# hrpan/tetris_mcts

Hardware: NVIDIA H100
Metric: mcts_sims_per_sec (higher is better)
Workload: dtype f32

## Files before the change

### tetris_mcts_b200/csrc/valuenet_tc.cuh

```cuda
#pragma once
#include <cuda_fp16.h>
#include "gmma.cuh"
#include "search_dev.cuh"
#include "valuenet_simt.cuh"

namespace b200 {

constexpr float TC_SCALE_A = 16.f, TC_SCALE_W = 64.f, TC_UNSCALE = 1.f / 1024.f;

__device__ __forceinline__ void wgmma_n64(float (&d)[32], uint64_t adesc, uint64_t bdesc, uint32_t accumulate) {
    asm volatile(
        "{\n.reg .pred p;\nsetp.ne.b32 p, %34, 0;\n"
        "wgmma.mma_async.sync.aligned.m64n64k16.f32.f16.f16 {"
        "%0,%1,%2,%3,%4,%5,%6,%7,%8,%9,%10,%11,%12,%13,%14,%15,"
        "%16,%17,%18,%19,%20,%21,%22,%23,%24,%25,%26,%27,%28,%29,%30,%31"
        "}, %32, %33, p, 1, 1, 0, 0;\n}"
        : "+f"(d[0]), "+f"(d[1]), "+f"(d[2]), "+f"(d[3]), "+f"(d[4]), "+f"(d[5]), "+f"(d[6]), "+f"(d[7]),
          "+f"(d[8]), "+f"(d[9]), "+f"(d[10]), "+f"(d[11]), "+f"(d[12]), "+f"(d[13]), "+f"(d[14]), "+f"(d[15]),
          "+f"(d[16]), "+f"(d[17]), "+f"(d[18]), "+f"(d[19]), "+f"(d[20]), "+f"(d[21]), "+f"(d[22]), "+f"(d[23]),
          "+f"(d[24]), "+f"(d[25]), "+f"(d[26]), "+f"(d[27]), "+f"(d[28]), "+f"(d[29]), "+f"(d[30]), "+f"(d[31])
        : "l"(adesc), "l"(bdesc), "r"(accumulate));
}
__device__ __forceinline__ void wgmma_n96(float (&d)[48], uint64_t adesc, uint64_t bdesc, uint32_t accumulate) {
    asm volatile(
        "{\n.reg .pred p;\nsetp.ne.b32 p, %50, 0;\n"
        "wgmma.mma_async.sync.aligned.m64n96k16.f32.f16.f16 {"
        "%0,%1,%2,%3,%4,%5,%6,%7,%8,%9,%10,%11,%12,%13,%14,%15,"
        "%16,%17,%18,%19,%20,%21,%22,%23,%24,%25,%26,%27,%28,%29,%30,%31,"
        "%32,%33,%34,%35,%36,%37,%38,%39,%40,%41,%42,%43,%44,%45,%46,%47"
        "}, %48, %49, p, 1, 1, 0, 0;\n}"
        : "+f"(d[0]), "+f"(d[1]), "+f"(d[2]), "+f"(d[3]), "+f"(d[4]), "+f"(d[5]), "+f"(d[6]), "+f"(d[7]),
          "+f"(d[8]), "+f"(d[9]), "+f"(d[10]), "+f"(d[11]), "+f"(d[12]), "+f"(d[13]), "+f"(d[14]), "+f"(d[15]),
          "+f"(d[16]), "+f"(d[17]), "+f"(d[18]), "+f"(d[19]), "+f"(d[20]), "+f"(d[21]), "+f"(d[22]), "+f"(d[23]),
          "+f"(d[24]), "+f"(d[25]), "+f"(d[26]), "+f"(d[27]), "+f"(d[28]), "+f"(d[29]), "+f"(d[30]), "+f"(d[31]),
          "+f"(d[32]), "+f"(d[33]), "+f"(d[34]), "+f"(d[35]), "+f"(d[36]), "+f"(d[37]), "+f"(d[38]), "+f"(d[39]),
          "+f"(d[40]), "+f"(d[41]), "+f"(d[42]), "+f"(d[43]), "+f"(d[44]), "+f"(d[45]), "+f"(d[46]), "+f"(d[47])
        : "l"(adesc), "l"(bdesc), "r"(accumulate));
}
__device__ __forceinline__ void wgmma_n128(float (&d)[64], uint64_t adesc, uint64_t bdesc, uint32_t accumulate) {
    asm volatile(
        "{\n.reg .pred p;\nsetp.ne.b32 p, %66, 0;\n"
        "wgmma.mma_async.sync.aligned.m64n128k16.f32.f16.f16 {"
        "%0,%1,%2,%3,%4,%5,%6,%7,%8,%9,%10,%11,%12,%13,%14,%15,"
        "%16,%17,%18,%19,%20,%21,%22,%23,%24,%25,%26,%27,%28,%29,%30,%31,"
        "%32,%33,%34,%35,%36,%37,%38,%39,%40,%41,%42,%43,%44,%45,%46,%47,"
        "%48,%49,%50,%51,%52,%53,%54,%55,%56,%57,%58,%59,%60,%61,%62,%63"
        "}, %64, %65, p, 1, 1, 0, 0;\n}"
        : "+f"(d[0]), "+f"(d[1]), "+f"(d[2]), "+f"(d[3]), "+f"(d[4]), "+f"(d[5]), "+f"(d[6]), "+f"(d[7]),
          "+f"(d[8]), "+f"(d[9]), "+f"(d[10]), "+f"(d[11]), "+f"(d[12]), "+f"(d[13]), "+f"(d[14]), "+f"(d[15]),
          "+f"(d[16]), "+f"(d[17]), "+f"(d[18]), "+f"(d[19]), "+f"(d[20]), "+f"(d[21]), "+f"(d[22]), "+f"(d[23]),
          "+f"(d[24]), "+f"(d[25]), "+f"(d[26]), "+f"(d[27]), "+f"(d[28]), "+f"(d[29]), "+f"(d[30]), "+f"(d[31]),
          "+f"(d[32]), "+f"(d[33]), "+f"(d[34]), "+f"(d[35]), "+f"(d[36]), "+f"(d[37]), "+f"(d[38]), "+f"(d[39]),
          "+f"(d[40]), "+f"(d[41]), "+f"(d[42]), "+f"(d[43]), "+f"(d[44]), "+f"(d[45]), "+f"(d[46]), "+f"(d[47]),
          "+f"(d[48]), "+f"(d[49]), "+f"(d[50]), "+f"(d[51]), "+f"(d[52]), "+f"(d[53]), "+f"(d[54]), "+f"(d[55]),
          "+f"(d[56]), "+f"(d[57]), "+f"(d[58]), "+f"(d[59]), "+f"(d[60]), "+f"(d[61]), "+f"(d[62]), "+f"(d[63])
        : "l"(adesc), "l"(bdesc), "r"(accumulate));
}
__device__ __forceinline__ void wgmma_n256(float (&d)[128], uint64_t adesc, uint64_t bdesc, uint32_t accumulate) {
    asm volatile(
        "{\n.reg .pred p;\nsetp.ne.b32 p, %130, 0;\n"
        "wgmma.mma_async.sync.aligned.m64n256k16.f32.f16.f16 {"
        "%0,%1,%2,%3,%4,%5,%6,%7,%8,%9,%10,%11,%12,%13,%14,%15,"
        "%16,%17,%18,%19,%20,%21,%22,%23,%24,%25,%26,%27,%28,%29,%30,%31,"
        "%32,%33,%34,%35,%36,%37,%38,%39,%40,%41,%42,%43,%44,%45,%46,%47,"
        "%48,%49,%50,%51,%52,%53,%54,%55,%56,%57,%58,%59,%60,%61,%62,%63,"
        "%64,%65,%66,%67,%68,%69,%70,%71,%72,%73,%74,%75,%76,%77,%78,%79,"
        "%80,%81,%82,%83,%84,%85,%86,%87,%88,%89,%90,%91,%92,%93,%94,%95,"
        "%96,%97,%98,%99,%100,%101,%102,%103,%104,%105,%106,%107,%108,%109,%110,%111,"
        "%112,%113,%114,%115,%116,%117,%118,%119,%120,%121,%122,%123,%124,%125,%126,%127"
        "}, %128, %129, p, 1, 1, 0, 0;\n}"
        : "+f"(d[0]), "+f"(d[1]), "+f"(d[2]), "+f"(d[3]), "+f"(d[4]), "+f"(d[5]), "+f"(d[6]), "+f"(d[7]),
          "+f"(d[8]), "+f"(d[9]), "+f"(d[10]), "+f"(d[11]), "+f"(d[12]), "+f"(d[13]), "+f"(d[14]), "+f"(d[15]),
          "+f"(d[16]), "+f"(d[17]), "+f"(d[18]), "+f"(d[19]), "+f"(d[20]), "+f"(d[21]), "+f"(d[22]), "+f"(d[23]),
          "+f"(d[24]), "+f"(d[25]), "+f"(d[26]), "+f"(d[27]), "+f"(d[28]), "+f"(d[29]), "+f"(d[30]), "+f"(d[31]),
          "+f"(d[32]), "+f"(d[33]), "+f"(d[34]), "+f"(d[35]), "+f"(d[36]), "+f"(d[37]), "+f"(d[38]), "+f"(d[39]),
          "+f"(d[40]), "+f"(d[41]), "+f"(d[42]), "+f"(d[43]), "+f"(d[44]), "+f"(d[45]), "+f"(d[46]), "+f"(d[47]),
          "+f"(d[48]), "+f"(d[49]), "+f"(d[50]), "+f"(d[51]), "+f"(d[52]), "+f"(d[53]), "+f"(d[54]), "+f"(d[55]),
          "+f"(d[56]), "+f"(d[57]), "+f"(d[58]), "+f"(d[59]), "+f"(d[60]), "+f"(d[61]), "+f"(d[62]), "+f"(d[63]),
          "+f"(d[64]), "+f"(d[65]), "+f"(d[66]), "+f"(d[67]), "+f"(d[68]), "+f"(d[69]), "+f"(d[70]), "+f"(d[71]),
          "+f"(d[72]), "+f"(d[73]), "+f"(d[74]), "+f"(d[75]), "+f"(d[76]), "+f"(d[77]), "+f"(d[78]), "+f"(d[79]),
          "+f"(d[80]), "+f"(d[81]), "+f"(d[82]), "+f"(d[83]), "+f"(d[84]), "+f"(d[85]), "+f"(d[86]), "+f"(d[87]),
          "+f"(d[88]), "+f"(d[89]), "+f"(d[90]), "+f"(d[91]), "+f"(d[92]), "+f"(d[93]), "+f"(d[94]), "+f"(d[95]),
          "+f"(d[96]), "+f"(d[97]), "+f"(d[98]), "+f"(d[99]), "+f"(d[100]), "+f"(d[101]), "+f"(d[102]), "+f"(d[103]),
          "+f"(d[104]), "+f"(d[105]), "+f"(d[106]), "+f"(d[107]), "+f"(d[108]), "+f"(d[109]), "+f"(d[110]), "+f"(d[111]),
          "+f"(d[112]), "+f"(d[113]), "+f"(d[114]), "+f"(d[115]), "+f"(d[116]), "+f"(d[117]), "+f"(d[118]), "+f"(d[119]),
          "+f"(d[120]), "+f"(d[121]), "+f"(d[122]), "+f"(d[123]), "+f"(d[124]), "+f"(d[125]), "+f"(d[126]), "+f"(d[127])
        : "l"(adesc), "l"(bdesc), "r"(accumulate));
}
__device__ __forceinline__ void split2(float x0, float x1, uint32_t &hi, uint32_t &lo) {
    const __half2 h = __floats2half2_rn(x0, x1);
    const float2 f = __half22float2(h);
    const __half2 l = __floats2half2_rn(x0 - f.x, x1 - f.y);
    hi = *reinterpret_cast<const uint32_t *>(&h); lo = *reinterpret_cast<const uint32_t *>(&l);
}

constexpr int TCC_WGS = 4;
constexpr int TCC_THREADS = TCC_WGS * 128;
constexpr int TCC_R = 144;
constexpr int TCC_WBLOCK = 2 * 2 * 96 * 16;
constexpr int TCC_WBYTES = 6 * TCC_WBLOCK;
constexpr int TCC_W1BYTES = 2 * 64 * 16;
constexpr int TCC_RUN = 4;
constexpr int TCC_ASLOT = 2 * 4 * TCC_R * 16;
constexpr int TCC_IMROWS = 192;
constexpr int TCC_IMSLOT = 2 * TCC_IMROWS * 16;
constexpr int TCC_OFF_W2 = 0;
constexpr int TCC_OFF_W3 = TCC_OFF_W2 + TCC_WBYTES;
constexpr int TCC_OFF_W1 = TCC_OFF_W3 + TCC_WBYTES;
constexpr int TCC_OFF_A1 = TCC_OFF_W1 + TCC_W1BYTES;
constexpr int TCC_OFF_IM = TCC_OFF_A1 + TCC_WGS * TCC_ASLOT;
constexpr int TCC_OFF_BIAS = TCC_OFF_IM + TCC_WGS * TCC_IMSLOT;
constexpr int TCC_OFF_KEY = TCC_OFF_BIAS + 96 * 4;
constexpr int TCC_SMEM = TCC_OFF_KEY + TCC_WGS * 32 * 4;
constexpr int ACT3_KCHUNKS = 224;
static_assert(TCC_SMEM <= 227 * 1024, "k_tc_conv shared memory");

struct TcWeights {
    const uint8_t *wc1;
    const uint8_t *wc2, *wc3;
    const uint8_t *wfc;
};

__device__ __forceinline__ size_t act3_off(int split, int n_tiles, int ridx, int kchunk) {
    return ((((size_t)split * n_tiles + (ridx >> 7)) * ACT3_KCHUNKS + kchunk) * 128 + (ridx & 127)) * 16;
}

__device__ __forceinline__ void issue_conv_layer(float (&d)[48], uint32_t a_addr, uint32_t w_addr) {
    const uint64_t a0 = gmma_desc(a_addr, TCC_R * 16, 128), b0 = gmma_desc(w_addr, 96 * 16, 128);
#pragma unroll
    for (int dy = 0; dy < 3; ++dy) {
#pragma unroll
        for (int h = 0; h < 2; ++h) {
            const uint32_t a_hi = 2 * h * TCC_R + dy * 8, a_lo = a_hi + 4 * TCC_R;
            const uint32_t b_hi = (dy * 2 + h) * (TCC_WBLOCK / 16), b_lo = b_hi + 2 * 96;
            wgmma_n96(d, a0 + a_hi, b0 + b_hi, (dy | h) ? 1u : 0u);
            wgmma_n96(d, a0 + a_hi, b0 + b_lo, 1u);
            wgmma_n96(d, a0 + a_lo, b0 + b_hi, 1u);
        }
    }
}

__device__ __forceinline__ void build_im2col3(uint8_t *im, const uint32_t *tab, int wt) {
    for (int p = wt; p < TCC_R; p += 128) {
        const int y = p >> 3, x = p & 7;
        uint32_t hv[9];
#pragma unroll
        for (int dy = 0; dy < 3; ++dy) {
            const uint32_t rw = tab[y + dy] >> x;
#pragma unroll
            for (int dx = 0; dx < 3; ++dx)
                hv[dy * 3 + dx] = ((rw >> dx) & 1u) * 0x3C00u | ((rw >> (16 + dx)) & 1u) * 0xBC00u;
        }
        *reinterpret_cast<uint4 *>(im + p * 16) =
            make_uint4(hv[0] | (hv[1] << 16), hv[2] | (hv[3] << 16), hv[4] | (hv[5] << 16), hv[6] | (hv[7] << 16));
        *reinterpret_cast<uint32_t *>(im + TCC_IMROWS * 16 + p * 16) = hv[8];
    }
}

__global__ void __launch_bounds__(TCC_THREADS, 1)
k_tc_conv(NetWeights W, TcWeights TW, const uint2 *req, const int32_t *n_req_ptr, const int32_t *first_ptr, const uint32_t *keys, int M, uint8_t *act3,
          int n_tiles, unsigned long long *prof) {
    extern __shared__ __align__(128) uint8_t smem[];
    float *sB = reinterpret_cast<float *>(smem + TCC_OFF_BIAS);
    const int t = threadIdx.x, wg = t >> 7, wt = t & 127, w = wt >> 5, lane = t & 31;
    for (int i = t; i < TCC_WBYTES / 16; i += TCC_THREADS) {
        reinterpret_cast<uint4 *>(smem + TCC_OFF_W2)[i] = reinterpret_cast<const uint4 *>(TW.wc2)[i];
        reinterpret_cast<uint4 *>(smem + TCC_OFF_W3)[i] = reinterpret_cast<const uint4 *>(TW.wc3)[i];
    }
    for (int i = t; i < TCC_W1BYTES / 16; i += TCC_THREADS) reinterpret_cast<uint4 *>(smem + TCC_OFF_W1)[i] = reinterpret_cast<const uint4 *>(TW.wc1)[i];
    for (int i = t; i < (TCC_OFF_BIAS - TCC_OFF_A1) / 16; i += TCC_THREADS) reinterpret_cast<uint4 *>(smem + TCC_OFF_A1)[i] = make_uint4(0, 0, 0, 0);
    if (t < 32) { sB[t] = W.b1[t] * TC_SCALE_A; sB[32 + t] = W.b2[t] * TC_SCALE_A; sB[64 + t] = W.b3[t] * TC_SCALE_A; }
    fence_async_smem();
    __syncthreads();
    const int first = first_ptr ? *first_ptr : 0;
    const int n_req = *n_req_ptr - first;
    const int n_workers = (int)gridDim.x * TCC_WGS, wid = (int)blockIdx.x * TCC_WGS + wg;
    const int n_runs = (n_req + TCC_RUN - 1) / TCC_RUN;
    int n_local = 0;
    for (int run = wid; run < n_runs; run += n_workers) n_local += min(TCC_RUN, n_req - run * TCC_RUN);
    auto board_of = [&](int i) -> int { return first + ((i / TCC_RUN) * n_workers + wid) * TCC_RUN + (i % TCC_RUN); };
    uint8_t *act = smem + TCC_OFF_A1 + wg * TCC_ASLOT, *im = smem + TCC_OFF_IM + wg * TCC_IMSLOT;
    uint32_t *sKey = reinterpret_cast<uint32_t *>(smem + TCC_OFF_KEY) + wg * 32;
    const uint32_t s_act = smem_u32(act), s_im = smem_u32(im);
    const uint32_t s_w1 = smem_u32(smem + TCC_OFF_W1), s_w2 = smem_u32(smem + TCC_OFF_W2), s_w3 = smem_u32(smem + TCC_OFF_W3);
    const int qd = lane & 3, rl = lane >> 2;
    constexpr float K23 = TC_UNSCALE * TC_SCALE_A, K1 = TC_SCALE_A / TC_SCALE_W;
    constexpr int SPLIT = 4 * TCC_R * 16;
    const bool do_prof = prof && blockIdx.x == 0 && t == 0;
    long long pacc[4] = {0, 0, 0, 0}, ptick = clock64();
    auto prof_t = [&](int k) { if (do_prof) { const long long n = clock64(); pacc[k] += n - ptick; ptick = n; } };
    auto fetch = [&](int i) -> uint32_t {
        if (i >= n_local || lane >= 12) return 0u;
        const uint2 rq = req[board_of(i)];
        return keys[((size_t)rq.x * M + (rq.y & 0x0fffffffu)) * KEY_WORDS + lane];
    };
    uint32_t kw = w == 0 ? fetch(0) : 0u;
    for (int i = 0; i < n_local; ++i) {
        const int ridx = board_of(i);
        if (w == 0) {
            const uint32_t rowpair = __shfl_sync(0xffffffffu, kw, (lane >> 1) & 15), pcs = __shfl_sync(0xffffffffu, kw, 10);
            uint32_t tab = (rowpair >> ((lane & 1) * 16)) & 0x3ffu;
#pragma unroll
            for (int k = 0; k < 4; ++k) {
                const uint32_t cell = (pcs >> (8 * k)) & 0xffu, pr = (cell * 205u) >> 11, pcol = cell - pr * 10u;
                tab |= (pr == (uint32_t)lane ? 1u : 0u) << (16 + pcol);
            }
            kw = fetch(i + 1);
            if (lane < 20) sKey[lane] = tab;
        }
        wg_sync(wg);
        build_im2col3(im, sKey, wt);
        fence_async_smem();
        wg_sync(wg);
        prof_t(0);
#pragma unroll 1
        for (int mt = 0; mt < 3; ++mt) {
            float d[32];
#pragma unroll
            for (int k = 0; k < 32; ++k) d[k] = 0.f;
            wgmma_fence();
            wgmma_n64(d, gmma_desc(s_im + mt * 1024, TCC_IMROWS * 16, 128), gmma_desc(s_w1, 64 * 16, 128), 0u);
            wgmma_commit();
            wgmma_wait<0>();
            fence_regs(d);
#pragma unroll
            for (int h = 0; h < 2; ++h) {
                const int r = mt * 64 + 16 * w + 8 * h + rl;
                if (r < TCC_R) {
#pragma unroll
                    for (int j = 0; j < 4; ++j) {
                        const int c = 8 * j + 2 * qd;
                        const float o0 = fmaxf(fmaf(d[4 * (j + 4) + 2 * h] + d[4 * j + 2 * h], K1, sB[c]), 0.f);
                        const float o1 = fmaxf(fmaf(d[4 * (j + 4) + 2 * h + 1] + d[4 * j + 2 * h + 1], K1, sB[c + 1]), 0.f);
                        uint32_t hi, lo;
                        split2(o0, o1, hi, lo);
                        uint8_t *dst = act + (j * TCC_R + r) * 16 + qd * 4;
                        *reinterpret_cast<uint32_t *>(dst) = hi;
                        *reinterpret_cast<uint32_t *>(dst + SPLIT) = lo;
                    }
                }
            }
        }
        fence_async_smem();
        wg_sync(wg);
        prof_t(1);
#pragma unroll 1
        for (int layer = 0; layer < 2; ++layer) {
            const float *bias = sB + 32 * (layer + 1);
#pragma unroll 1
            for (int mt = 0; mt < 2; ++mt) {
                float d[48];
#pragma unroll
                for (int k = 0; k < 48; ++k) d[k] = 0.f;
                wgmma_fence();
                issue_conv_layer(d, s_act + mt * 1024, layer ? s_w3 : s_w2);
                wgmma_commit();
                wgmma_wait<0>();
                fence_regs(d);
#pragma unroll
                for (int h = 0; h < 2; ++h) {
                    const int y = mt * 8 + 2 * w + h, x = rl;
#pragma unroll
                    for (int j = 0; j < 4; ++j) {
                        float o[2];
#pragma unroll
                        for (int e = 0; e < 2; ++e) {
                            const int k = 4 * j + 2 * h + e;
                            const float s1 = __shfl_down_sync(0xffffffffu, d[16 + k], 4), s2 = __shfl_down_sync(0xffffffffu, d[32 + k], 8);
                            o[e] = fmaxf(fmaf((s2 + s1) + d[k], K23, bias[8 * j + 2 * qd + e]), 0.f);
                        }
                        uint32_t hi, lo;
                        split2(o[0], o[1], hi, lo);
                        if (layer == 0) {
                            if (x < 6) {
                                uint8_t *dst = act + (j * TCC_R + y * 8 + x) * 16 + qd * 4;
                                *reinterpret_cast<uint32_t *>(dst) = hi;
                                *reinterpret_cast<uint32_t *>(dst + SPLIT) = lo;
                            }
                        } else if (y < 14 && x < 4) {
                            const int kc = (y * 4 + x) * 4 + j;
                            *reinterpret_cast<uint32_t *>(act3 + act3_off(0, n_tiles, ridx, kc) + qd * 4) = hi;
                            *reinterpret_cast<uint32_t *>(act3 + act3_off(1, n_tiles, ridx, kc) + qd * 4) = lo;
                        }
                    }
                }
            }
            fence_async_smem();
            wg_sync(wg);
            prof_t(2 + layer);
        }
    }
    if (do_prof) for (int k = 0; k < 4; ++k) atomicAdd(&prof[k], (unsigned long long)pacc[k]);
}

constexpr int TCF_CONSUMERS = 2;
constexpr int TCF_PRODUCER = TCF_CONSUMERS * 4;
constexpr int TCF_THREADS = TCF_CONSUMERS * 128 + 32;
constexpr int TCF_STAGES = 8;
constexpr int TCF_A_BYTES = 2 * 128 * 16;
constexpr int TCF_B_BYTES = 2 * 256 * 16;
constexpr int TCF_STAGE = 2 * TCF_A_BYTES + 2 * TCF_B_BYTES;
constexpr int TCF_KBLOCKS = 112;
constexpr int TCF_OFF_BAR = TCF_STAGES * TCF_STAGE;
constexpr int TCF_OFF_EPI = TCF_OFF_BAR + 256;
static_assert(2 * TCF_STAGES * 8 <= 256, "barrier block overflows into the epilogue constants");
constexpr int TCF_SMEM = TCF_OFF_EPI + (256 * 3 + 8) * 4;
static_assert(TCF_SMEM <= 227 * 1024, "k_tc_fc shared memory");

__global__ void __launch_bounds__(TCF_THREADS, 1)
k_tc_fc(NetWeights W, TcWeights TW, const uint8_t *act3, int n_tiles_alloc, const uint2 *req, const int32_t *n_req_ptr, float2 *eval_out) {
    extern __shared__ __align__(128) uint8_t smem[];
    uint64_t *full = reinterpret_cast<uint64_t *>(smem + TCF_OFF_BAR);
    uint64_t *empty = full + TCF_STAGES;
    float *sBias = reinterpret_cast<float *>(smem + TCF_OFF_EPI), *sWo = sBias + 256, *sTail = sWo + 512;
    const int t = threadIdx.x, warp = t >> 5, lane = t & 31;
    for (int i = t; i < 256; i += TCF_THREADS) { sBias[i] = W.bfc1[i]; sWo[i] = W.wout[i]; sWo[256 + i] = W.wout[256 + i]; }
    if (t < 2) { sTail[t] = W.bout[t]; sTail[2 + t] = W.ub[t]; sTail[4 + t] = W.lb[t]; }
    if (t == 0) {
        for (int i = 0; i < TCF_STAGES; ++i) { mbar_init(&full[i], 1); mbar_init(&empty[i], TCF_CONSUMERS); }
        fence_barrier_init();
    }
    __syncthreads();
    const int n_req = *n_req_ptr;
    const int n_tiles = (n_req + 127) >> 7;
    if (warp == TCF_PRODUCER) {
        if (lane == 0) {
            int stage = 0; uint32_t ph = 0;
            for (int tile = blockIdx.x; tile < n_tiles; tile += gridDim.x) {
                for (int j = 0; j < TCF_KBLOCKS; ++j) {
                    mbar_wait(&empty[stage], ph ^ 1);
                    mbar_expect_tx(&full[stage], TCF_STAGE);
                    uint8_t *dst = smem + stage * TCF_STAGE;
#pragma unroll
                    for (int s = 0; s < 2; ++s) {
                        bulk_g2s(dst + s * TCF_A_BYTES, act3 + (((size_t)s * n_tiles_alloc + tile) * ACT3_KCHUNKS + 2 * j) * 2048, TCF_A_BYTES, &full[stage]);
                        bulk_g2s(dst + 2 * TCF_A_BYTES + s * TCF_B_BYTES, TW.wfc + ((size_t)s * TCF_KBLOCKS + j) * TCF_B_BYTES, TCF_B_BYTES, &full[stage]);
                    }
                    if (++stage == TCF_STAGES) { stage = 0; ph ^= 1; }
                }
            }
        }
    } else {
        const int wg = t >> 7, w = warp & 3, qd = lane & 3, rl = lane >> 2;
        int stage = 0; uint32_t ph = 0;
        for (int tile = blockIdx.x; tile < n_tiles; tile += gridDim.x) {
            float d[128];
#pragma unroll
            for (int k = 0; k < 128; ++k) d[k] = 0.f;
            int prev = -1;
            for (int j = 0; j < TCF_KBLOCKS; ++j) {
                mbar_wait(&full[stage], ph);
                const uint32_t sbase = smem_u32(smem + stage * TCF_STAGE);
                wgmma_fence();
#pragma unroll
                for (int term = 0; term < 3; ++term) {
                    const int sa = term == 1 ? 1 : 0, sb = term == 0 ? 1 : 0;
                    const uint64_t ad = gmma_desc(sbase + sa * TCF_A_BYTES + wg * 1024, 128 * 16, 128);
                    const uint64_t bd = gmma_desc(sbase + 2 * TCF_A_BYTES + sb * TCF_B_BYTES, 256 * 16, 128);
                    wgmma_n256(d, ad, bd, (j | term) ? 1u : 0u);
                }
                wgmma_commit();
                wgmma_wait<1>();
                if (prev >= 0 && (t & 127) == 0) mbar_arrive(&empty[prev]);
                prev = stage;
                if (++stage == TCF_STAGES) { stage = 0; ph ^= 1; }
            }
            wgmma_wait<0>();
            fence_regs(d);
            if ((t & 127) == 0) mbar_arrive(&empty[prev]);
            float p0[2] = {0.f, 0.f}, p1[2] = {0.f, 0.f};
#pragma unroll
            for (int j = 0; j < 32; ++j)
#pragma unroll
                for (int h = 0; h < 2; ++h)
#pragma unroll
                    for (int e = 0; e < 2; ++e) {
                        const int c = 8 * j + 2 * qd + e;
                        const float hv = fmaxf(d[4 * j + 2 * h + e] * TC_UNSCALE + sBias[c], 0.f);
                        p0[h] = fmaf(hv, sWo[c], p0[h]); p1[h] = fmaf(hv, sWo[256 + c], p1[h]);
                    }
#pragma unroll
            for (int h = 0; h < 2; ++h) {
                p0[h] += __shfl_xor_sync(0xffffffffu, p0[h], 1); p1[h] += __shfl_xor_sync(0xffffffffu, p1[h], 1);
                p0[h] += __shfl_xor_sync(0xffffffffu, p0[h], 2); p1[h] += __shfl_xor_sync(0xffffffffu, p1[h], 2);
                const int ridx = tile * 128 + wg * 64 + 16 * w + 8 * h + rl;
                if (qd == 0 && ridx < n_req) {
                    const float x0 = p0[h] + sTail[0], x1 = p1[h] + sTail[1];
                    const float s0 = 1.f / (1.f + expf(-x0)), s1 = 1.f / (1.f + expf(-x1));
                    const uint2 rq = req[ridx];
                    eval_out[(size_t)rq.x * 8 + (rq.y >> 28)] =
                        make_float2(__fadd_rn(__fmul_rn(s0, sTail[2]), sTail[4]), __fadd_rn(__fmul_rn(s1, sTail[3]), sTail[5]));
                }
            }
        }
    }
}

struct TcState {
    uint8_t *d_w = nullptr;
    TcWeights TW{};
    uint8_t *d_act3 = nullptr; size_t tiles = 0;
};

static inline void host_split2(float x, uint16_t *o) {
    __half h1 = __float2half_rn(x);
    __half h2 = __float2half_rn(x - __half2float(h1));
    memcpy(&o[0], &h1, 2); memcpy(&o[1], &h2, 2);
}
static inline float host_half_f(uint16_t h) { __half x; memcpy(&x, &h, 2); return __half2float(x); }

static inline bool tc_split_fits(const float *x, size_t n) {
    for (size_t i = 0; i < n; ++i)
        if (!(fabsf(x[i]) * TC_SCALE_W <= 65504.f)) return false;
    return true;
}
static bool tc_weights_fit(const float *w) {
    const float *c1w = w, *c2w = w + 288 + 32, *c3w = c2w + 9216 + 32, *f1w = c3w + 9216 + 32;
    return tc_split_fits(c1w, 288) && tc_split_fits(c2w, 9216) && tc_split_fits(c3w, 9216) && tc_split_fits(f1w, (size_t)256 * 1792);
}

static int tc_prepare(void **state, const float *w, cudaStream_t stream) {
    TcState *st = (TcState *)*state;
    if (!st) { st = new TcState(); *state = st; }
    const float *c1w = w, *c2w = w + 288 + 32, *c3w = c2w + 9216 + 32, *f1w = c3w + 9216 + 32;
    const size_t fc_bytes = (size_t)2 * TCF_KBLOCKS * TCF_B_BYTES;
    std::vector<uint8_t> h(TCC_W1BYTES + 2 * (size_t)TCC_WBYTES + fc_bytes);
    uint16_t *p1 = reinterpret_cast<uint16_t *>(h.data());
    uint16_t *p2 = reinterpret_cast<uint16_t *>(h.data() + TCC_W1BYTES), *p3 = reinterpret_cast<uint16_t *>(h.data() + TCC_W1BYTES + TCC_WBYTES);
    uint16_t *pf = reinterpret_cast<uint16_t *>(h.data() + TCC_W1BYTES + 2 * (size_t)TCC_WBYTES);
    for (int c2 = 0; c2 < 2; ++c2)
        for (int n = 0; n < 32; ++n)
            for (int e = 0; e < 8; ++e) {
                const int tap = 8 * c2 + e;
                uint16_t s2[2] = {0, 0};
                if (tap < 9) host_split2(c1w[n * 9 + tap] * TC_SCALE_W, s2);
                for (int s = 0; s < 2; ++s) p1[((size_t)c2 * 64 + s * 32 + n) * 8 + e] = s2[s];
            }
    for (int layer = 0; layer < 2; ++layer) {
        const float *cw = layer ? c3w : c2w;
        uint16_t *dst = layer ? p3 : p2;
        for (int dy = 0; dy < 3; ++dy)
            for (int hh = 0; hh < 2; ++hh)
                for (int c2 = 0; c2 < 2; ++c2)
                    for (int dx = 0; dx < 3; ++dx)
                        for (int n = 0; n < 32; ++n)
                            for (int e = 0; e < 8; ++e) {
                                int ci = 16 * hh + 8 * c2 + e;
                                uint16_t s2[2];
                                host_split2(cw[(n * 32 + ci) * 9 + dy * 3 + dx] * TC_SCALE_W, s2);
                                for (int s = 0; s < 2; ++s)
                                    dst[(((((size_t)(dy * 2 + hh)) * 2 + s) * 2 + c2) * 96 + dx * 32 + n) * 8 + e] = s2[s];
                            }
    }
    for (int j = 0; j < TCF_KBLOCKS; ++j)
        for (int c2 = 0; c2 < 2; ++c2)
            for (int n = 0; n < 256; ++n)
                for (int e = 0; e < 8; ++e) {
                    int kp = j * 16 + c2 * 8 + e, p = kp >> 5, c = kp & 31;
                    uint16_t s2[2];
                    host_split2(f1w[(size_t)n * 1792 + c * 56 + p] * TC_SCALE_W, s2);
                    for (int s = 0; s < 2; ++s) pf[((((size_t)s * TCF_KBLOCKS + j) * 2 + c2) * 256 + n) * 8 + e] = s2[s];
                }
    if (!st->d_w && cudaMalloc(&st->d_w, h.size()) != cudaSuccess) return 1;
    if (cudaMemcpyAsync(st->d_w, h.data(), h.size(), cudaMemcpyHostToDevice, stream) != cudaSuccess) return 1;
    if (cudaStreamSynchronize(stream) != cudaSuccess) return 1;
    st->TW.wc1 = st->d_w; st->TW.wc2 = st->d_w + TCC_W1BYTES; st->TW.wc3 = st->TW.wc2 + TCC_WBYTES; st->TW.wfc = st->TW.wc3 + TCC_WBYTES;
    if (cudaFuncSetAttribute(k_tc_conv, cudaFuncAttributeMaxDynamicSharedMemorySize, TCC_SMEM) != cudaSuccess) return 1;
    if (cudaFuncSetAttribute(k_tc_fc, cudaFuncAttributeMaxDynamicSharedMemorySize, TCF_SMEM) != cudaSuccess) return 1;
    return 0;
}

static int tc_ensure_act3(TcState *st, size_t max_rows, cudaStream_t stream) {
    size_t tiles = (max_rows + 127) / 128;
    if (st->tiles >= tiles) return 0;
    if (st->d_act3) { cudaStreamSynchronize(stream); cudaFree(st->d_act3); st->d_act3 = nullptr; }
    size_t bytes = (size_t)2 * tiles * ACT3_KCHUNKS * 2048;
    if (cudaMalloc(&st->d_act3, bytes) != cudaSuccess) return 1;
    cudaMemsetAsync(st->d_act3, 0, bytes, stream);
    st->tiles = tiles;
    return 0;
}

static void tc_destroy(void *state) {
    TcState *st = (TcState *)state;
    if (!st) return;
    cudaFree(st->d_w); cudaFree(st->d_act3);
    delete st;
}

}
```

Before: 8.654 million.

## Compute conv3 only on valid output region with transposed act2 layout and n32 wgmma

Conv layer 3 previously ran the same full 2x m64n96 tile pass as conv2, which produced outputs later discarded (only 14x4 of the positions are kept). It now writes conv2 outputs into a separate transposed, bank-padded act2 buffer and computes conv3 as a single m64 tile with three m64n32 accumulators, one per dx tap. This drops the second M-tile and the shuffle reductions. It costs extra shared memory, an in-register rotation to transpose the layout, and a reordered conv3 weight packing on the host.

```diff
diff --git a/tetris_mcts_b200/csrc/valuenet_tc.cuh b/tetris_mcts_b200/csrc/valuenet_tc.cuh
--- a/tetris_mcts_b200/csrc/valuenet_tc.cuh
+++ b/tetris_mcts_b200/csrc/valuenet_tc.cuh
@@ -8,6 +8,16 @@
 
 constexpr float TC_SCALE_A = 16.f, TC_SCALE_W = 64.f, TC_UNSCALE = 1.f / 1024.f;
 
+__device__ __forceinline__ void wgmma_n32(float (&d)[16], uint64_t adesc, uint64_t bdesc, uint32_t accumulate) {
+    asm volatile(
+        "{\n.reg .pred p;\nsetp.ne.b32 p, %18, 0;\n"
+        "wgmma.mma_async.sync.aligned.m64n32k16.f32.f16.f16 {"
+        "%0,%1,%2,%3,%4,%5,%6,%7,%8,%9,%10,%11,%12,%13,%14,%15"
+        "}, %16, %17, p, 1, 1, 0, 0;\n}"
+        : "+f"(d[0]), "+f"(d[1]), "+f"(d[2]), "+f"(d[3]), "+f"(d[4]), "+f"(d[5]), "+f"(d[6]), "+f"(d[7]),
+          "+f"(d[8]), "+f"(d[9]), "+f"(d[10]), "+f"(d[11]), "+f"(d[12]), "+f"(d[13]), "+f"(d[14]), "+f"(d[15])
+        : "l"(adesc), "l"(bdesc), "r"(accumulate));
+}
 __device__ __forceinline__ void wgmma_n64(float (&d)[32], uint64_t adesc, uint64_t bdesc, uint32_t accumulate) {
     asm volatile(
         "{\n.reg .pred p;\nsetp.ne.b32 p, %34, 0;\n"
@@ -99,9 +109,15 @@
 constexpr int TCC_R = 144;
 constexpr int TCC_WBLOCK = 2 * 2 * 96 * 16;
 constexpr int TCC_WBYTES = 6 * TCC_WBLOCK;
+constexpr int TCC_W3BLOCK = 2 * 32 * 16;
+static_assert(36 * TCC_W3BLOCK == TCC_WBYTES, "conv3 weight layout");
 constexpr int TCC_W1BYTES = 2 * 64 * 16;
 constexpr int TCC_RUN = 4;
 constexpr int TCC_ASLOT = 2 * 4 * TCC_R * 16;
+constexpr int TCC_R2 = 98;
+constexpr int TCC_A2SPLIT = 4 * TCC_R2 * 16 + 16;
+constexpr int TCC_A2SLOT = 2 * TCC_A2SPLIT;
+static_assert((TCC_R2 * 4) % 32 == 8 && (TCC_A2SPLIT / 4) % 32 == 4, "act2 bank layout");
 constexpr int TCC_IMROWS = 192;
 constexpr int TCC_IMSLOT = 2 * TCC_IMROWS * 16;
 constexpr int TCC_OFF_W2 = 0;
@@ -109,7 +125,8 @@
 constexpr int TCC_OFF_W1 = TCC_OFF_W3 + TCC_WBYTES;
 constexpr int TCC_OFF_A1 = TCC_OFF_W1 + TCC_W1BYTES;
 constexpr int TCC_OFF_IM = TCC_OFF_A1 + TCC_WGS * TCC_ASLOT;
-constexpr int TCC_OFF_BIAS = TCC_OFF_IM + TCC_WGS * TCC_IMSLOT;
+constexpr int TCC_OFF_A2 = TCC_OFF_IM + TCC_WGS * TCC_IMSLOT;
+constexpr int TCC_OFF_BIAS = TCC_OFF_A2 + TCC_WGS * TCC_A2SLOT;
 constexpr int TCC_OFF_KEY = TCC_OFF_BIAS + 96 * 4;
 constexpr int TCC_SMEM = TCC_OFF_KEY + TCC_WGS * 32 * 4;
 constexpr int ACT3_KCHUNKS = 224;
@@ -125,7 +142,7 @@
     return ((((size_t)split * n_tiles + (ridx >> 7)) * ACT3_KCHUNKS + kchunk) * 128 + (ridx & 127)) * 16;
 }
 
-__device__ __forceinline__ void issue_conv_layer(float (&d)[48], uint32_t a_addr, uint32_t w_addr) {
+__device__ __forceinline__ void issue_conv2(float (&d)[48], uint32_t a_addr, uint32_t w_addr) {
     const uint64_t a0 = gmma_desc(a_addr, TCC_R * 16, 128), b0 = gmma_desc(w_addr, 96 * 16, 128);
 #pragma unroll
     for (int dy = 0; dy < 3; ++dy) {
@@ -136,6 +153,24 @@
             wgmma_n96(d, a0 + a_hi, b0 + b_hi, (dy | h) ? 1u : 0u);
             wgmma_n96(d, a0 + a_hi, b0 + b_lo, 1u);
             wgmma_n96(d, a0 + a_lo, b0 + b_hi, 1u);
+        }
+    }
+}
+
+__device__ __forceinline__ void issue_conv3(float (&d)[3][16], uint32_t a_addr, uint32_t w_addr) {
+    const uint64_t a0 = gmma_desc(a_addr, TCC_R2 * 16, 128), b0 = gmma_desc(w_addr, 32 * 16, 128);
+#pragma unroll
+    for (int dy = 0; dy < 3; ++dy) {
+#pragma unroll
+        for (int h = 0; h < 2; ++h) {
+#pragma unroll
+            for (int dx = 0; dx < 3; ++dx) {
+                const uint32_t a_hi = 2 * h * TCC_R2 + 16 * dx + dy, a_lo = a_hi + TCC_A2SPLIT / 16;
+                const uint32_t b_hi = ((dx * 3 + dy) * 2 + h) * 2 * (TCC_W3BLOCK / 16), b_lo = b_hi + TCC_W3BLOCK / 16;
+                wgmma_n32(d[dx], a0 + a_hi, b0 + b_hi, (dy | h) ? 1u : 0u);
+                wgmma_n32(d[dx], a0 + a_hi, b0 + b_lo, 1u);
+                wgmma_n32(d[dx], a0 + a_lo, b0 + b_hi, 1u);
+            }
         }
     }
 }
@@ -179,9 +214,9 @@
     int n_local = 0;
     for (int run = wid; run < n_runs; run += n_workers) n_local += min(TCC_RUN, n_req - run * TCC_RUN);
     auto board_of = [&](int i) -> int { return first + ((i / TCC_RUN) * n_workers + wid) * TCC_RUN + (i % TCC_RUN); };
-    uint8_t *act = smem + TCC_OFF_A1 + wg * TCC_ASLOT, *im = smem + TCC_OFF_IM + wg * TCC_IMSLOT;
+    uint8_t *act = smem + TCC_OFF_A1 + wg * TCC_ASLOT, *act2 = smem + TCC_OFF_A2 + wg * TCC_A2SLOT, *im = smem + TCC_OFF_IM + wg * TCC_IMSLOT;
     uint32_t *sKey = reinterpret_cast<uint32_t *>(smem + TCC_OFF_KEY) + wg * 32;
-    const uint32_t s_act = smem_u32(act), s_im = smem_u32(im);
+    const uint32_t s_act = smem_u32(act), s_act2 = smem_u32(act2), s_im = smem_u32(im);
     const uint32_t s_w1 = smem_u32(smem + TCC_OFF_W1), s_w2 = smem_u32(smem + TCC_OFF_W2), s_w3 = smem_u32(smem + TCC_OFF_W3);
     const int qd = lane & 3, rl = lane >> 2;
     constexpr float K23 = TC_UNSCALE * TC_SCALE_A, K1 = TC_SCALE_A / TC_SCALE_W;
@@ -245,50 +280,83 @@
         wg_sync(wg);
         prof_t(1);
 #pragma unroll 1
-        for (int layer = 0; layer < 2; ++layer) {
-            const float *bias = sB + 32 * (layer + 1);
-#pragma unroll 1
-            for (int mt = 0; mt < 2; ++mt) {
-                float d[48];
-#pragma unroll
-                for (int k = 0; k < 48; ++k) d[k] = 0.f;
-                wgmma_fence();
-                issue_conv_layer(d, s_act + mt * 1024, layer ? s_w3 : s_w2);
-                wgmma_commit();
-                wgmma_wait<0>();
-                fence_regs(d);
-#pragma unroll
-                for (int h = 0; h < 2; ++h) {
-                    const int y = mt * 8 + 2 * w + h, x = rl;
-#pragma unroll
-                    for (int j = 0; j < 4; ++j) {
-                        float o[2];
-#pragma unroll
-                        for (int e = 0; e < 2; ++e) {
-                            const int k = 4 * j + 2 * h + e;
-                            const float s1 = __shfl_down_sync(0xffffffffu, d[16 + k], 4), s2 = __shfl_down_sync(0xffffffffu, d[32 + k], 8);
-                            o[e] = fmaxf(fmaf((s2 + s1) + d[k], K23, bias[8 * j + 2 * qd + e]), 0.f);
-                        }
-                        uint32_t hi, lo;
-                        split2(o[0], o[1], hi, lo);
-                        if (layer == 0) {
-                            if (x < 6) {
-                                uint8_t *dst = act + (j * TCC_R + y * 8 + x) * 16 + qd * 4;
-                                *reinterpret_cast<uint32_t *>(dst) = hi;
-                                *reinterpret_cast<uint32_t *>(dst + SPLIT) = lo;
-                            }
-                        } else if (y < 14 && x < 4) {
-                            const int kc = (y * 4 + x) * 4 + j;
-                            *reinterpret_cast<uint32_t *>(act3 + act3_off(0, n_tiles, ridx, kc) + qd * 4) = hi;
-                            *reinterpret_cast<uint32_t *>(act3 + act3_off(1, n_tiles, ridx, kc) + qd * 4) = lo;
-                        }
-                    }
-                }
-            }
-            fence_async_smem();
-            wg_sync(wg);
-            prof_t(2 + layer);
-        }
+        for (int mt = 0; mt < 2; ++mt) {
+            float d[48];
+#pragma unroll
+            for (int k = 0; k < 48; ++k) d[k] = 0.f;
+            wgmma_fence();
+            issue_conv2(d, s_act + mt * 1024, s_w2);
+            wgmma_commit();
+            wgmma_wait<0>();
+            fence_regs(d);
+#pragma unroll
+            for (int h = 0; h < 2; ++h) {
+                const int y = mt * 8 + 2 * w + h, x = rl;
+                uint32_t v[8];
+#pragma unroll
+                for (int j = 0; j < 4; ++j) {
+                    float o[2];
+#pragma unroll
+                    for (int e = 0; e < 2; ++e) {
+                        const int k = 4 * j + 2 * h + e;
+                        const float s1 = __shfl_down_sync(0xffffffffu, d[16 + k], 4), s2 = __shfl_down_sync(0xffffffffu, d[32 + k], 8);
+                        o[e] = fmaxf(fmaf((s2 + s1) + d[k], K23, sB[32 + 8 * j + 2 * qd + e]), 0.f);
+                    }
+                    split2(o[0], o[1], v[j], v[4 + j]);
+                }
+#pragma unroll
+                for (int b = 1; b < 8; b <<= 1) {
+                    uint32_t r[8];
+#pragma unroll
+                    for (int k = 0; k < 8; ++k) r[k] = (x & b) ? v[(k + b) & 7] : v[k];
+#pragma unroll
+                    for (int k = 0; k < 8; ++k) v[k] = r[k];
+                }
+                if (x < 6) {
+#pragma unroll
+                    for (int k = 0; k < 8; ++k) {
+                        const int i = (k + x) & 7;
+                        *reinterpret_cast<uint32_t *>(act2 + (i >> 2) * TCC_A2SPLIT + ((i & 3) * TCC_R2 + x * 16 + y) * 16 + qd * 4) = v[k];
+                    }
+                }
+            }
+        }
+        fence_async_smem();
+        wg_sync(wg);
+        prof_t(2);
+        {
+            float d[3][16];
+#pragma unroll
+            for (int k = 0; k < 16; ++k) d[0][k] = d[1][k] = d[2][k] = 0.f;
+            wgmma_fence();
+            issue_conv3(d, s_act2, s_w3);
+            wgmma_commit();
+            wgmma_wait<0>();
+            fence_regs(d[0]); fence_regs(d[1]); fence_regs(d[2]);
+            const int x = w;
+#pragma unroll
+            for (int h = 0; h < 2; ++h) {
+                const int y = 8 * h + rl;
+#pragma unroll
+                for (int j = 0; j < 4; ++j) {
+                    float o[2];
+#pragma unroll
+                    for (int e = 0; e < 2; ++e) {
+                        const int k = 4 * j + 2 * h + e;
+                        o[e] = fmaxf(fmaf((d[2][k] + d[1][k]) + d[0][k], K23, sB[64 + 8 * j + 2 * qd + e]), 0.f);
+                    }
+                    uint32_t hi, lo;
+                    split2(o[0], o[1], hi, lo);
+                    if (y < 14) {
+                        const int kc = (y * 4 + x) * 4 + j;
+                        *reinterpret_cast<uint32_t *>(act3 + act3_off(0, n_tiles, ridx, kc) + qd * 4) = hi;
+                        *reinterpret_cast<uint32_t *>(act3 + act3_off(1, n_tiles, ridx, kc) + qd * 4) = lo;
+                    }
+                }
+            }
+        }
+        wg_sync(wg);
+        prof_t(3);
     }
     if (do_prof) for (int k = 0; k < 4; ++k) atomicAdd(&prof[k], (unsigned long long)pacc[k]);
 }
@@ -436,22 +504,21 @@
                 if (tap < 9) host_split2(c1w[n * 9 + tap] * TC_SCALE_W, s2);
                 for (int s = 0; s < 2; ++s) p1[((size_t)c2 * 64 + s * 32 + n) * 8 + e] = s2[s];
             }
-    for (int layer = 0; layer < 2; ++layer) {
-        const float *cw = layer ? c3w : c2w;
-        uint16_t *dst = layer ? p3 : p2;
-        for (int dy = 0; dy < 3; ++dy)
-            for (int hh = 0; hh < 2; ++hh)
-                for (int c2 = 0; c2 < 2; ++c2)
-                    for (int dx = 0; dx < 3; ++dx)
-                        for (int n = 0; n < 32; ++n)
-                            for (int e = 0; e < 8; ++e) {
-                                int ci = 16 * hh + 8 * c2 + e;
-                                uint16_t s2[2];
-                                host_split2(cw[(n * 32 + ci) * 9 + dy * 3 + dx] * TC_SCALE_W, s2);
-                                for (int s = 0; s < 2; ++s)
-                                    dst[(((((size_t)(dy * 2 + hh)) * 2 + s) * 2 + c2) * 96 + dx * 32 + n) * 8 + e] = s2[s];
+    for (int dy = 0; dy < 3; ++dy)
+        for (int hh = 0; hh < 2; ++hh)
+            for (int c2 = 0; c2 < 2; ++c2)
+                for (int dx = 0; dx < 3; ++dx)
+                    for (int n = 0; n < 32; ++n)
+                        for (int e = 0; e < 8; ++e) {
+                            int ci = 16 * hh + 8 * c2 + e, tap = dy * 3 + dx;
+                            uint16_t s2[2], s3[2];
+                            host_split2(c2w[(n * 32 + ci) * 9 + tap] * TC_SCALE_W, s2);
+                            host_split2(c3w[(n * 32 + ci) * 9 + tap] * TC_SCALE_W, s3);
+                            for (int s = 0; s < 2; ++s) {
+                                p2[(((((size_t)(dy * 2 + hh)) * 2 + s) * 2 + c2) * 96 + dx * 32 + n) * 8 + e] = s2[s];
+                                p3[((((((size_t)(dx * 3 + dy)) * 2 + hh) * 2 + s) * 2 + c2) * 32 + n) * 8 + e] = s3[s];
                             }
-    }
+                        }
     for (int j = 0; j < TCF_KBLOCKS; ++j)
         for (int c2 = 0; c2 < 2; ++c2)
             for (int n = 0; n < 256; ++n)
```

After: 9.287 million (median of 6 runs). +7.3%, better.
